# cgrigis/drynx

Hardware: AMD Instinct MI355X
Metric: end-to-end query latency + range-proof verifications/sec, logreg on 1e6 records (higher is better)
Workload: dtype bn254-exact/fp64

## Files before the change

### drynx_amd/native/__init__.py

```python
from __future__ import annotations

import ctypes
import os
import threading

import numpy as np

import torch

_HERE = os.path.dirname(os.path.abspath(__file__))
LIB_PATH = os.environ.get("DRYNX_NATIVE_LIB") or os.path.join(_HERE, "libdrynx_native.so")

_lib = None


def _load():
    global _lib
    if _lib is not None:
        return _lib
    if not os.path.exists(LIB_PATH):
        if os.environ.get("DRYNX_AUTOBUILD", "1") == "1":
            from . import build as _b

            _b.build()
        else:
            raise ImportError(f"{LIB_PATH} missing: run `python -m drynx_amd.native.build`")
    _lib = ctypes.CDLL(LIB_PATH)
    _declare(_lib)
    return _lib


_P = ctypes.c_void_p
_I = ctypes.c_int
_L = ctypes.c_int64

_SIGS = {
    "dx_fp_to_mont": [_I, _P, _P, _P, _L],
    "dx_fp_from_mont": [_I, _P, _P, _P, _L],
    "dx_fr_arith": [_I, _P, _I, _P, _P, _P, _L, _L],
    "dx_fr_dot_chunks": [_I, _P, _P, _P, _I, _P, _L, _L, _L],
    "dx_fr_seg_sum": [_I, _P, _P, _P, _P, _L],
    "dx_rp_challenges": [_I, _P, _P, _P, _P, _P, _P, _L],
    "dx_g1_fb_table": [_I, _P, _P, _P, _P, _L],
    "dx_g1_fb_mul": [_I, _P, _P, _P, _P, _L],
    "dx_g1_fb_mul_i64": [_I, _P, _P, _P, _P, _L],
    "dx_g1_fb_mul_idx": [_I, _P, _P, _P, _P, _P, _L],
    "dx_g1_mul": [_I, _P, _P, _P, _P, _L, _I, _I],
    "dx_g1_add": [_I, _P, _P, _P, _P, _L, _I, _I],
    "dx_g1_to_affine": [_I, _P, _P, _P, _L],
    "dx_g1_from_affine": [_I, _P, _P, _P, _L],
    "dx_g1_eq": [_I, _P, _P, _P, _P, _L],
    "dx_g1_on_curve": [_I, _P, _P, _P, _L],
    "dx_g1_sum_chunks": [_I, _P, _P, _P, _L, _L, _L],
    "dx_elgamal_encrypt": [_I, _P, _P, _P, _P, _P, _P, _P, _L],
    "dx_bsgs_build": [_I, _P, _P, _L, _P, _P, _L],
    "dx_bsgs_solve": [_I, _P, _P, _P, _P, _P, _L, _L, _L, _L, _P, _P, _L],
    "dx_g2_fb_table": [_I, _P, _P, _P, _P, _L],
    "dx_g2_fb_mul": [_I, _P, _P, _P, _P, _P, _L],
    "dx_g2_mul": [_I, _P, _P, _P, _P, _L, _I],
    "dx_g2_on_curve": [_I, _P, _P, _P, _L],
    "dx_miller_loop": [_I, _P, _P, _P, _P, _L],
    "dx_final_exp": [_I, _P, _P, _P, _L],
    "dx_pairing": [_I, _P, _P, _P, _P, _L],
    "dx_gt_mul": [_I, _P, _P, _P, _P, _L],
    "dx_gt_inv": [_I, _P, _P, _P, _L],
    "dx_prg_glv": [_I, _P, _P, ctypes.c_uint32, _P, _P, _P, _L],
    "dx_prg_bits": [_I, _P, _P, ctypes.c_uint32, _I, _P, _L],
    "dx_batched_copy": [_I, _P, _P, _P, _I, _L],
    "dx_copy_out": [_I, _P, _P, _P, _I, _L, _I],
    "dx_host_device_ptr": [_P, _P],
    "dx_rows_all": [_I, _P, _P, _P, _I, _L, _P],
    "dx_gt_pow": [_I, _P, _P, _P, _P, _L, _I],
    "dx_gt_eq": [_I, _P, _P, _P, _P, _L],
    "dx_gt_fb_table": [_I, _P, _P, _P, _P, _L],
    "dx_gt_fb_pow": [_I, _P, _P, _P, _P, _P, _L],
    "dx_gt_prod_chunks": [_I, _P, _P, _P, _L, _L, _L],
    "dx_version": [],
    "dx_lr_moments": [_P, _P, _P, _L, _I, _P, _I, _I],
    "dx_lr_gd_k2": [_P, _P, _P, _I, ctypes.c_double, ctypes.c_double, ctypes.c_double, _I, ctypes.c_double,
                    ctypes.c_double, ctypes.c_double, _P],
    "dx_random_scalars": [_I, _P, _P, ctypes.c_uint32, _P, _L],
    "dx_sha256_chunks": [_I, _P, _P, _L, _L, _P],
    "dx_hash_to_g1": [_I, _P, _P, _P, _L, _P, _L],
    "dx_lr_encode": [_P, _P, _L, _L, _I, _P, _P, _P, ctypes.c_double, ctypes.c_double, _P, _I, _I],
    "dx_lr_reduce": [_P, _P, _L, _L, _L, _P],
    "dx_lr_encode_upper": [_P, _P, _L, _L, _I, _P, _P, _P, ctypes.c_double, ctypes.c_double, _P, _I, _I],
    "dx_lr_reduce_pack": [_P, _P, _L, _I, _I, _L, ctypes.c_double, _P, _P],
    "dx_lr_encode_multi": [_P, _P, _L, _L, _I, _P, _P, _P, _L, _I, ctypes.c_double, _P, _I, _I, _I],
    "dx_lr_reduce_pack_multi": [_P, _P, _L, _I, _I, _I, _L, ctypes.c_double, _P, _P],
    "dx_g1_mul_glv256": [_P, _P, _P, _P, _P, _L, _I, _I, _I],
    "dx_glv_split": [_I, _P, _P, _P, _L],
    "dx_gt_t2_compress": [_I, _P, _P, _P, _P, _L],
    "dx_g2_x_compress": [_I, _P, _P, _P, _P, _P, _L],
    "dx_g2_x_decompress": [_I, _P, _P, _P, _P, _P, _L],
    "dx_gt_t2_decompress": [_I, _P, _P, _P, _L],
    "dx_gt_slice_prod": [_I, _P, _P, _P, _P, _P, _P, _L],
    "dx_gt_chunk_weight": [_I, _P, _P, _P, _P, _P, _P, _P, _L],
    "dx_g1_mul_glv": [_P, _P, _P, _P, _P, _L, _I],
    "dx_rp_u_joint_split": [_I, _P, _P, _P, _P, _L, _I, _I, _L, _I, _P, _P],
    "dx_bucket_bounds": [_I, _P, _P, _L, _L, _P, _P],
    "dx_slice_desc": [_I, _P, _P, _P, _P, _I, _L, _L, _P, _P],
    "dx_lane_slices": [_I, _P, _P, _P, _P, _P, _P, _L, _P, _P],
    "dx_g1_slice_sum": [_I, _P, _P, _P, _P, _P, _P, _L],
    "dx_rp_prove_a": [_I, _P, _P, _P, _P, _P, _P, _L, _I, _I],
    "dx_rp_prove_a_tab": [_I, _P, _P, _P, _P, _P, _P, _P, _L, _I, _I, _I],
    "dx_g2_fb4_table": [_I, _P, _P, _P, _P, _L],
    "dx_g2_fb4_mul": [_I, _P, _P, _P, _P, _P, _L],
    "dx_gt_fb4_table": [_I, _P, _P, _P, _P, _L],
    "dx_gt_fb4_pow": [_I, _P, _P, _P, _P, _P, _L],
    "dx_gt_cyclotomic": [_I, _P, _P, _P, _L],
    "dx_gt_membership": [_I, _P, _P, _P, _L],
    "dx_g1_horner_host": [_P, _P, _L, _I, _I],
    "dx_fp_sqrt_host": [_P, _P, _P, _P, _L],
    "dx_g2_chunk_weight": [_I, _P, _P, _P, _P, _P, _P, _P, _L],
    "dx_g2_subgroup": [_I, _P, _P, _P, _L],
    "dx_limbs_canonical": [_I, _P, _P, _I, _P, _L],
    "dx_g1j_on_curve": [_I, _P, _P, _P, _L],
    "dx_fold_steps": [],
    "dx_rp_coeffs": [_P, _P, _P, _L],
    "dx_int_moments": [_I, _P, _P, _L, _I, _P, _L, _P, _I, _P, _P],
    "dx_sha256_rows": [_I, _P, _P, _L, _L, _L, _L, _P],
    "dx_sha256_segments": [_I, _P, _P, _L, _L, _L, _P],
    "dx_g1_aff_to_uv": [_I, _P, _P, _L],
    "dx_rp_ncoeffs": [_P, _P, _P, _P, _L],
    "dx_rp_accum_n": [_P, _P, _P, _P, _P, _L, _L, _I, _I],
    "dx_ufold_coop_raw": [_P, _P, _P, _P, _P, _L, _L, _L],
    "dx_gt_frob8": [_I, _P, _P, _P, _L],
    "dx_gls6_entries": [],
    "dx_g2_gls6_table": [_I, _P, _P, _P, _P, _L],
    "dx_g2_gls6_mul": [_I, _P, _P, _P, _P, _P, _L],
    "dx_gt_gls6_table": [_I, _P, _P, _P, _P, _L],
    "dx_gt_gls6_pow": [_I, _P, _P, _P, _P, _P, _L],
    "dx_rp_prove_a_gls6": [_I, _P, _P, _P, _P, _P, _P, _P, _L, _I, _I],
    "dx_g2_joint_table": [_I, _P, _P, _P, _L],
    "dx_g2_joint_table_signed": [_I, _P, _P, _P, _P, _L],
    "dx_rp_u_group": [_I, _P, _P, _P, _P, _P, _P, _P, _L, _I, _L, _I, _I, _L, _P, _P],
    "dx_rp_u_joint": [_I, _P, _P, _P, _P, _L, _I, _I, _L, _P],
    "dx_g2_slice_sum": [_I, _P, _P, _P, _P, _P, _P, _L, _I, _L],
    "dx_g2_horner": [_I, _P, _P, _P, _I, _I, _I, _L, _L],
    "dx_rp_msm_uv": [_I, _P, _P, _P, _L, _I, _L],
    "dx_msm_keys": [_I, _P, _P, _P, _L, _L, _I, _I, _P, _P],
    "dx_gls8_entries": [],
    "dx_g2_gls8_table": [_I, _P, _P, _P, _P, _L],
    "dx_gt_gls8_table": [_I, _P, _P, _P, _P, _L, _P, _L],
    "dx_g2_gls8_mul": [_I, _P, _P, _P, _P, _P, _L],
    "dx_rp_prove_a_gls8": [_I, _P, _P, _P, _P, _P, _P, _P, _L, _I, _I, _I, _P],
    "dx_gt16_entries": [],
    "dx_gt16_table": [_I, _P, _P, _P, _P],
}


def _declare(lib):
    for name, args in _SIGS.items():
        fn = getattr(lib, name)
        fn.argtypes = args
        fn.restype = ctypes.c_int


def lib():
    return _load()


def loaded_path() -> str:
    _load()
    return LIB_PATH


_keep = threading.local()


def _ptr(t: torch.Tensor | None):
    if t is None:
        return None
    assert t.is_contiguous(), "native ops need contiguous tensors"
    held = getattr(_keep, "held", None)
    if held is None:
        held = _keep.held = []
    held.append(t)
    return ctypes.c_void_p(t.data_ptr())

# ... 1106 lines not shown
        raw = _bn.random_scalars(n, device)
    ab = raw[:, :2].contiguous()
    a = torch.zeros_like(raw)
    b = torch.zeros_like(raw)
    a[:, 0] = ab[:, 0]
    b[:, 0] = ab[:, 1]
    rho = fr_arith(FR_ADD, a, fr_arith(FR_MUL, b, _glv_const("lambda", device)))
    return ab, rho


def g1_mul_glv(pts_jac: torch.Tensor, ab: torch.Tensor) -> torch.Tensor:
    n = _rows(ab, 2)
    np_ = _rows(pts_jac, 24)
    assert np_ in (1, n)
    if not ab.is_cuda:
        a = torch.zeros((n, 8), dtype=torch.int32)
        b = torch.zeros((n, 8), dtype=torch.int32)
        a[:, 0], b[:, 0] = ab[:, 0], ab[:, 1]
        rho = fr_arith(FR_ADD, a, fr_arith(FR_MUL, b, _glv_const("lambda", "cpu")))
        return g1_mul(pts_jac, rho)
    out = torch.empty((n, 24), dtype=torch.int32, device=ab.device)
    _, s = _ctx(pts_jac, ab)
    rc = _raw_call("dx_g1_mul_glv", s, _ptr(pts_jac.contiguous()), _ptr(ab.contiguous()),
                   _ptr(_glv_const("beta", ab.device)), _ptr(out), n, int(np_ == 1 and n > 1))
    if rc:
        raise RuntimeError(f"dx_g1_mul_glv failed rc={rc}")
    return out


def g1_aff_to_uv_(aff: torch.Tensor) -> torch.Tensor:
    g, s = _ctx(aff)
    _call("dx_g1_aff_to_uv", g, s, _ptr(aff), _rows(aff, 16))
    return aff


FOLD_P_ALIGN = 8


def rp_fold_ncoeffs(V_aff: torch.Tensor) -> torch.Tensor:
    m = _rows(V_aff, 32)
    assert V_aff.is_cuda and V_aff.is_contiguous()
    steps = _load().dx_fold_steps()
    img = torch.empty((steps * 8 * m * 4,), dtype=torch.int32, device=V_aff.device)
    scratch = torch.empty((2 * steps * 4 * m * 4,), dtype=torch.int32, device=V_aff.device)
    _, s = _ctx(V_aff)
    _call("dx_rp_ncoeffs", s, _ptr(V_aff), _ptr(img), _ptr(scratch), m)
    return img


def rp_fold_accum_n(img: torch.Tensor, UV: torch.Tensor, V_aff: torch.Tensor, period: int, G: int,
                    K: int = 4) -> torch.Tensor:
    m = _rows(V_aff, 32)
    assert _rows(UV, 16) == G * period and period >= m and period % (64 * K * FOLD_P_ALIGN) == 0
    assert img.numel() == _load().dx_fold_steps() * 8 * m * 4
    fb = torch.empty((G * period // (64 * K), 96), dtype=torch.int32, device=UV.device)
    _, s = _ctx(img, UV, V_aff)
    _call("dx_rp_accum_n", s, _ptr(img), _ptr(UV), _ptr(V_aff), _ptr(fb), m, period, G, K)
    return fb


def rp_fold_accum_coop_raw(coef: torch.Tensor, P_aff: torch.Tensor, V_aff: torch.Tensor, period: int,
                           G: int) -> torch.Tensor:
    m = _rows(V_aff, 32)
    n = G * period
    assert _rows(P_aff, 16) == n and period >= m and period % 64 == 0
    assert coef.numel() == _load().dx_fold_steps() * 12 * m * 4
    f = torch.empty((n, 96), dtype=torch.int32, device=P_aff.device)
    _, s = _ctx(coef, P_aff, V_aff)
    _call("dx_ufold_coop_raw", s, _ptr(coef), _ptr(P_aff), _ptr(V_aff), _ptr(f), m, period, n)
    x = f.view(64, n // 64, 96)
    while x.shape[0] > 1:
        x = _gt_prod_level(x, 8)
    return x.view(n // 64, 96)


def gt_frob8(a: torch.Tensor, out: torch.Tensor | None = None) -> torch.Tensor:
    out = torch.empty_like(a) if out is None else out
    assert out.is_contiguous() and out.shape == a.shape
    g, s = _ctx(a)
    _call("dx_gt_frob8", g, s, _ptr(a.contiguous()), _ptr(out), _rows(a, 96))
    return out


def rp_fold_coeffs(V_aff: torch.Tensor) -> torch.Tensor:
    m = _rows(V_aff, 32)
    assert V_aff.is_cuda and V_aff.is_contiguous()
    coef = torch.empty((_load().dx_fold_steps() * 12 * m * 4,), dtype=torch.int32, device=V_aff.device)
    _, s = _ctx(V_aff)
    _call("dx_rp_coeffs", s, _ptr(V_aff), _ptr(coef), m)
    return coef


G2_JOINT_ENTRIES = 15


def g2_joint_table(V_aff: torch.Tensor, sign: torch.Tensor | None = None) -> torch.Tensor:
    m = _rows(V_aff, 32)
    out = torch.empty((m * G2_JOINT_ENTRIES, 32), dtype=torch.int32, device=V_aff.device)
    if sign is None:
        g, s = _ctx(V_aff)
        _call("dx_g2_joint_table", g, s, _ptr(V_aff.contiguous()), _ptr(out), m)
        return out
    assert sign.dtype == torch.int32 and sign.numel() == m
    g, s = _ctx(V_aff, sign)
    _call("dx_g2_joint_table_signed", g, s, _ptr(V_aff.contiguous()), _ptr(sign.contiguous()), _ptr(out), m)
    return out


def rp_u_joint(table: torch.Tensor, ab: torch.Tensor, n_groups: int, G: int, L: int, out: torch.Tensor,
               pad: int, pos: torch.Tensor | None = None) -> torch.Tensor:
    assert _rows(table, 32) == n_groups * L * G2_JOINT_ENTRIES and _rows(ab, 2) == G * n_groups * L
    assert out.is_contiguous() and pad >= n_groups
    if pos is None:
        assert _rows(out, 32) >= (G - 1) * pad + n_groups
    else:
        assert pos.dtype == torch.int64 and pos.numel() == G * n_groups and pos.device == out.device
    g, s = _ctx(table, ab, out)
    n = G * n_groups
    sp = 1 if (not g or n >= 131072) else (2 if n >= 65536 else 4)
    sp = min(sp, L)
    if sp > 1:
        tmp = torch.empty((n * sp, 48), dtype=torch.int32, device=out.device)
        _call("dx_rp_u_joint_split", g, s, _ptr(table), _ptr(ab.contiguous()), _ptr(out), n_groups, G, L, pad, sp,
              _ptr(tmp), _ptr(pos))
        return out
    _call("dx_rp_u_joint", g, s, _ptr(table), _ptr(ab.contiguous()), _ptr(out), n_groups, G, L, pad, _ptr(pos))
    return out


def rp_u_group_lanes(n: int, on_gpu: bool) -> int:
    if not on_gpu:
        return 1
    sp = 1
    while sp < 16 and n * sp < 32768:
        sp *= 2
    return sp


def rp_u_group(table: torch.Tensor, split: torch.Tensor, idx: torch.Tensor, start: torch.Tensor,
               length: torch.Tensor, G: int, nq: int, S: int, out: torch.Tensor, pad: int,
               pos: torch.Tensor | None = None, sp: int | None = None) -> torch.Tensor:
    ng = start.numel()
    assert _rows(table, 32) == G * nq * G2_JOINT_ENTRIES and _rows(split, 9) * S >= nq
    assert idx.dtype == torch.int32 and start.dtype == torch.int64 and length.dtype == torch.int32
    assert length.numel() == ng and out.is_contiguous() and pad >= ng
    if pos is None:
        assert _rows(out, 32) >= (G - 1) * pad + ng
    else:
        assert pos.dtype == torch.int64 and pos.numel() == G * ng and pos.device == out.device
    g, s = _ctx(table, split, idx, start, length, out)
    if sp is None:
        sp = rp_u_group_lanes(G * ng, bool(g))
    assert sp >= 1 and 64 % sp == 0
    tmp = None if g else torch.empty((G * ng * sp, 48), dtype=torch.int32)
    _call("dx_rp_u_group", g, s, _ptr(table), _ptr(split.contiguous()), _ptr(idx), _ptr(start), _ptr(length),
          _ptr(out), ng, G, nq, S, sp, pad, _ptr(pos), _ptr(tmp))
    return out


_gt_one_cache: dict = {}


def gt_one(device) -> torch.Tensor:
    key = str(device)
    if key not in _gt_one_cache:
        from ..crypto import bn254 as _bn

        t = np.zeros((1, 96), dtype=np.uint32)
        t[0, :8] = _bn.ints_to_limbs([_bn.mont(1)])[0]
        _gt_one_cache[key] = _bn.publish(_bn.to_tensor(t, device))
    return _gt_one_cache[key]


def _pow2_scalar(c: int) -> torch.Tensor:
    t = torch.zeros((1, 8), dtype=torch.int32)
    t[0, c // 32] = 1 << (c % 32)
    return t


def _finish_prod_on_host(parts: torch.Tensor) -> torch.Tensor:
    cur = parts.view(-1, 1, 96)
    while cur.shape[0] > 256:
        cur = _gt_prod_level(cur, 8)
    return gt_prod(cur.cpu(), chunk=4).view(1, 96)


def _gt_prod_level(x: torch.Tensor, ch: int) -> torch.Tensor:
    n_items, n_groups = x.shape[0], x.shape[1]
    n_chunks = (n_items + ch - 1) // ch
    out = torch.empty((n_chunks, n_groups, 96), dtype=torch.int32, device=x.device)
    g, s = _ctx(x)
    _call("dx_gt_prod_chunks", g, s, _ptr(x.contiguous()), _ptr(out), n_items, n_groups, ch)
    return out


from .msm import (G2_CHUNK, capture_keep, check_overflow, g1_msm, g1_msm_device, g1_msm_finish,
                  g1_msm_grouped, g1_msm_launch, g1_msm_plan, g1_slice_sum, g2_chunk_weight, g2_msm_device,
                  g2_msm_finish, g2_msm_launch, g2_msm_run, g2_slice_sum, gt_chunk_weight, gt_slice_prod, me_window,
                  multi_exp_device, multi_exp_grouped, multi_exp_grouped_finish, multi_exp_plan, rp_msm_uv)
```

### drynx_amd/native/msm.py

```python
from __future__ import annotations

import threading

import numpy as np

import torch

from . import (_call, _ctx, _gt_prod_level, _pow2_scalar, _ptr, _raw_call, _rows, _upload, g1_mul, gt_mul, gt_one,
               gt_pow, gt_prod)

_ME_SLICE = 8
G2_CHUNK = 32


def gt_slice_prod(src: torch.Tensor, idx, start: torch.Tensor, length: torch.Tensor) -> torch.Tensor:
    n = start.numel()
    out = torch.empty((n, 96), dtype=torch.int32, device=src.device)
    g, s = _ctx(src, idx, start, length)
    _call("dx_gt_slice_prod", g, s, _ptr(src), _ptr(idx), _ptr(start), _ptr(length), _ptr(out), n)
    return out


def g1_slice_sum(src: torch.Tensor, idx, start: torch.Tensor, length: torch.Tensor) -> torch.Tensor:
    n = start.numel()
    out = torch.empty((n, 24), dtype=torch.int32, device=src.device)
    g, s = _ctx(src, idx, start, length)
    _call("dx_g1_slice_sum", g, s, _ptr(src), _ptr(idx), _ptr(start), _ptr(length), _ptr(out), n)
    return out


def g2_slice_sum(src: torch.Tensor, idx, start: torch.Tensor, length: torch.Tensor, src_aff: bool,
                 idx_mod: int = 0) -> torch.Tensor:
    n = start.numel()
    assert src.shape[-1] == (32 if src_aff else 48) and (idx is None or idx.dtype == torch.int32)
    assert start.dtype == torch.int64 and length.dtype == torch.int32
    out = torch.empty((n, 48), dtype=torch.int32, device=src.device)
    g, s = _ctx(src, idx, start, length)
    _call("dx_g2_slice_sum", g, s, _ptr(src), _ptr(idx), _ptr(start), _ptr(length), _ptr(out), n, int(src_aff),
          int(idx_mod))
    return out


def gt_chunk_weight(B: torch.Tensor, d: torch.Tensor, start: torch.Tensor, length: torch.Tensor,
                    base: torch.Tensor) -> torch.Tensor:
    n = start.numel()
    out = torch.empty((n, 96), dtype=torch.int32, device=B.device)
    g, s = _ctx(B, d, start, length, base)
    _call("dx_gt_chunk_weight", g, s, _ptr(B.contiguous()), _ptr(d.contiguous()), _ptr(start), _ptr(length),
          _ptr(base), _ptr(out), n)
    return out


def g2_chunk_weight(B_jac: torch.Tensor, d: torch.Tensor, start: torch.Tensor, length: torch.Tensor,
                    base: torch.Tensor) -> torch.Tensor:
    n = start.numel()
    assert B_jac.shape[-1] == 48 and d.dtype == torch.int32 and start.dtype == torch.int64
    assert length.dtype == torch.int32 and base.dtype == torch.int32 and base.numel() == n
    out = torch.empty((n, 48), dtype=torch.int32, device=B_jac.device)
    g, s = _ctx(B_jac, d, start, length, base)
    _call("dx_g2_chunk_weight", g, s, _ptr(B_jac.contiguous()), _ptr(d.contiguous()), _ptr(start), _ptr(length),
          _ptr(base), _ptr(out), n)
    return out


def _gt_ops(a: torch.Tensor, items: torch.Tensor, item_split: tuple | None = None):
    n = a.shape[0]
    it = items.to(torch.int64)
    if item_split is not None:
        sp, q = item_split
        it = torch.where(it < sp, it % n, (it - sp) % q)
    else:
        it = it % n
    it = it.contiguous()
    return (lambda st, ln: gt_slice_prod(a, it, st, ln)), (lambda cur, st, ln: gt_slice_prod(cur, None, st, ln))


def _g1_ops(P_jac: torch.Tensor, items: torch.Tensor):
    P_jac, it = P_jac.contiguous(), items.to(torch.int64)
    return (lambda st, ln: g1_slice_sum(P_jac, it, st, ln)), (lambda cur, st, ln: g1_slice_sum(cur, None, st, ln))


def _g2_ops(P_aff: torch.Tensor, items: torch.Tensor, m: int):
    return (lambda st, ln: g2_slice_sum(P_aff, items, st, ln, True, m)), \
        (lambda cur, st, ln: g2_slice_sum(cur, None, st, ln, False))


def _group_arg(group, n: int, dev):
    if group is None:
        return None, 0
    if isinstance(group, int):
        return None, group
    assert group.numel() == n
    return group.to(device=dev, dtype=torch.int32).contiguous(), 0


def _runs(k: torch.Tensor, group, n_groups: int, W: int, c: int):
    dev = k.device
    n = k.shape[0]
    nb = (W << c) * n_groups
    assert n * W < 2 ** 31 and nb < 2 ** 31 - 1
    keys = torch.empty(n * W, dtype=torch.int32, device=dev)
    items = torch.empty(n * W, dtype=torch.int32, device=dev)
    grp, gstride = _group_arg(group, n, dev)
    g, s = _ctx(k, keys)
    _call("dx_msm_keys", g, s, _ptr(k.contiguous()), _ptr(grp), gstride, n, c, W, _ptr(keys), _ptr(items))
    k2, order = torch.sort(keys)
    items = items.index_select(0, order)
    bounds = torch.zeros((2, nb), dtype=torch.int64, device=dev)
    g, s = _ctx(k2)
    _call("dx_bucket_bounds", g, s, _ptr(k2), keys.numel(), nb, _ptr(bounds[0]), _ptr(bounds[1]))
    return items, bounds[0], bounds[1]


def _segment_passes(counts, first=None):
    passes = []
    c = np.asarray(counts, dtype=np.int64)
    while c.size and c.max() > 1:
        n_sl = (c + _ME_SLICE - 1) // _ME_SLICE
        if first is None:
            first = np.cumsum(c) - c
        b = np.repeat(np.arange(c.size), n_sl)
        k = np.arange(b.size) - (np.cumsum(n_sl) - n_sl)[b]
        passes.append((first[b] + k * _ME_SLICE, np.minimum(c[b] - k * _ME_SLICE, _ME_SLICE)))
        c, first = n_sl, None
    return passes


def _segment_passes_dev(counts, dev, first_slice: int | None = None):
    passes = []
    c = np.asarray(counts, dtype=np.int64)
    while c.size and c.max() > 1:
        sl = first_slice if (first_slice and not passes) else _ME_SLICE
        n_sl = (c + sl - 1) // sl
        total = int(n_sl.sum())
        meta = np.stack([np.cumsum(c) - c, c, np.cumsum(n_sl) - n_sl])
        m_dev = _upload(meta, dev)
        start = torch.empty(total, dtype=torch.int64, device=dev)
        ln = torch.empty(total, dtype=torch.int32, device=dev)
        g, s = _ctx(m_dev)
        _call("dx_slice_desc", g, s, _ptr(m_dev[0]), _ptr(m_dev[1]), _ptr(m_dev[2]), sl, c.size, total, _ptr(start),
              _ptr(ln))
        passes.append((start, ln))
        c = n_sl
    return passes


def _counted_plan(k: torch.Tensor, group, n_groups: int, W: int, c: int, first_slice: int | None = None) -> dict:
    dev = k.device
    items, first, end = _runs(k, group, n_groups, W, c)
    counts = (end - first).cpu().numpy().astype(np.int64)
    bk = np.flatnonzero(counts)
    passes = _segment_passes_dev(counts[bk], dev, first_slice)
    if bk.size and not passes:
        passes = [(torch.arange(bk.size, device=dev), torch.ones(bk.size, dtype=torch.int32, device=dev))]
    return {"item": items[: int(counts.sum())], "bk": bk, "passes": passes, "W": W, "c": c}


# ... 125 lines not shown
    gws, counts = np.unique(bk // 256, return_counts=True)
    return {"sc": _upload(sc, dev), "gws": gws,
            "passes": [(_upload(st, dev), _upload(ln.astype("int32"), dev)) for st, ln in _segment_passes(counts)]}


def _g1_weigh(h: dict, cur: torch.Tensor, wp: dict):
    cur = g1_mul(cur, wp["sc"])
    for st, ln in wp["passes"]:
        cur = g1_slice_sum(cur, None, st, ln)
    h["S_w"], h["gws"] = cur, wp["gws"]


def _g2_chunk(n_buckets: int) -> int:
    ch = G2_CHUNK
    while ch > 4 and n_buckets // ch < 16384:
        ch //= 2
    return ch


def _chunk_weight_plan(bk, c: int, dev) -> dict:
    chunk = _g2_chunk(bk.size)
    dig = bk & ((1 << c) - 1)
    gw = bk >> c
    ck = gw * ((1 << c) // chunk + 1) + dig // chunk
    first = np.flatnonzero(np.r_[True, ck[1:] != ck[:-1]])
    clen = np.diff(np.r_[first, bk.size])
    gwf = gw[first]
    gstart = np.flatnonzero(np.r_[True, gwf[1:] != gwf[:-1]])
    gws, gcounts = gwf[gstart], np.diff(np.r_[gstart, gwf.size])
    return {"d": _upload(dig.astype("int32"), dev),
            "chunks": (_upload(first.astype(np.int64), dev), _upload(clen.astype(np.int32), dev),
                       _upload(((dig[first] // chunk) * chunk).astype(np.int32), dev)),
            "gws": _upload(gws.astype(np.int64), dev), "gpasses": _segment_passes_dev(gcounts, dev)}


def _g2_weigh(cur, wp: dict, S: torch.Tensor) -> torch.Tensor:
    cur = g2_chunk_weight(cur, wp["d"], *wp["chunks"])
    for st, ln in wp["gpasses"]:
        cur = g2_slice_sum(cur, None, st, ln, False)
    S.index_copy_(0, wp["gws"], cur)
    return S


def _me_windows(h: dict, cur, bk, n_groups: int, W: int, c: int, dev):
    digit_sc = torch.zeros((bk.size, 8), dtype=torch.int32)
    digit_sc[:, 0] = torch.from_numpy((bk & ((1 << c) - 1)).astype("int32"))
    bkp = gt_pow(cur, _upload(digit_sc.numpy(), dev))
    D = 1 << c
    g, w, d = bk // (W * D), (bk >> c) % W, bk & (D - 1)
    slot = _upload(d * (n_groups * W) + g * W + w, dev)
    win = gt_one(dev).repeat(D * n_groups * W, 1)
    win[slot] = bkp
    win = win.view(D, n_groups * W, 96)
    if torch.device(dev).type == "cuda":
        while win.shape[0] > 32:
            win = _gt_prod_level(win, 8)
    h["win"] = win
    h["G"] = n_groups


def me_window(groups: tuple, lo: int = 8, hi: int = 16) -> tuple:
    def cost(c):
        return sum(r * -(-b // c) for r, b in groups) + 3 * sum(-(-b // c) for _, b in groups) * (1 << c)
    c = min(range(lo, hi + 1), key=cost)
    return max(-(-b // c) for _, b in groups), c


def multi_exp_plan(k: torch.Tensor, group, n_groups: int, W: int = 8, c: int = 8):
    return _counted_plan(k, group, n_groups, W, c)


def multi_exp_grouped(a: torch.Tensor, k: torch.Tensor, group, n_groups: int, W: int = 8, c: int = 8,
                      plan: dict | None = None):
    if plan is None:
        plan = _counted_plan(k, group, n_groups, W, c)
    h = {"G": n_groups, "W": W, "c": c, "win": None}
    if plan["bk"].size:
        cur = _reduce(plan["passes"], _gt_ops(a, plan["item"]))
        _me_windows(h, cur, plan["bk"], n_groups, W, c, a.device)
    return h


def multi_exp_device(a: torch.Tensor, k: torch.Tensor, group, groups: tuple, W: int | None = None,
                     c: int | None = None, item_split: tuple | None = None) -> dict:
    dev = a.device
    G = len(groups)
    if c is None:
        W, c = me_window(tuple(groups))
    B, lay, overflow = _device_buckets(k, group, groups, W, c, _ME_SLICE, lambda items: _gt_ops(a, items, item_split))
    if "gtw" not in lay:
        lay["gtw"] = _chunk_weight_plan(lay["used"], c, dev)
    wp = lay["gtw"]
    cur = gt_chunk_weight(B, wp["d"], *wp["chunks"])
    for st, ln in wp["gpasses"]:
        cur = gt_slice_prod(cur, None, st, ln)
    win = gt_one(dev).repeat(G * W, 1)
    win.index_copy_(0, wp["gws"], cur)
    return {"G": G, "W": W, "c": c, "win": win.view(1, G * W, 96), "overflow": overflow}


def multi_exp_grouped_finish(h) -> torch.Tensor:
    G, W = h["G"], h["W"]
    if h["win"] is None:
        return gt_one("cpu").repeat(G, 1)
    S_w = gt_prod(h["win"].cpu(), chunk=64).view(G, W, 96)
    acc = S_w[:, W - 1].contiguous()
    sh = _pow2_scalar(h["c"]).expand(G, 8).contiguous()
    for w in range(W - 2, -1, -1):
        acc = gt_mul(gt_pow(acc, sh), S_w[:, w].contiguous())
    return acc


def g1_msm(P_jac: torch.Tensor, k: torch.Tensor, bits: int = 256) -> torch.Tensor:
    return g1_msm_grouped(P_jac, k, None, 1, bits)


def g1_msm_grouped(P_jac: torch.Tensor, k: torch.Tensor, group: torch.Tensor | None, n_groups: int,
                   bits: int = 256) -> torch.Tensor:
    return g1_msm_finish(g1_msm_launch(P_jac, k, group, n_groups, bits))


def g1_msm_plan(k: torch.Tensor, group, n_groups: int, bits: int = 256):
    if not k.shape[0]:
        return None
    return _counted_plan(k, group, n_groups, (bits + 7) // 8, 8)


def g1_msm_launch(P_jac: torch.Tensor, k: torch.Tensor, group: torch.Tensor | None, n_groups: int,
                  bits: int = 256, plan: dict | None = None) -> dict:
    assert P_jac.shape[0] == k.shape[0]
    assert group is None or isinstance(group, int) or group.numel() == k.shape[0]
    W = (bits + 7) // 8
    h = {"n_groups": n_groups, "W": W, "S_w": None}
    if P_jac.shape[0] == 0:
        return h
    if plan is None:
        plan = _counted_plan(k, group, n_groups, W, 8)
    bk = plan["bk"]
    if bk.size:
        cur = _reduce(plan["passes"], _g1_ops(P_jac, plan["item"]))
        _g1_weigh(h, cur, _g1_weight_plan(bk, P_jac.device))
    return h


def g1_msm_device(P_jac: torch.Tensor, k: torch.Tensor, group, groups: tuple, bits: int = 256) -> dict:
    W = (bits + 7) // 8
    B, lay, overflow = _device_buckets(k, group, groups, W, 8, _ME_SLICE, lambda items: _g1_ops(P_jac, items))
    h = {"n_groups": len(groups), "W": W, "S_w": None, "overflow": overflow}
    if "g1w" not in lay:
        lay["g1w"] = _g1_weight_plan(lay["used"], P_jac.device)
    _g1_weigh(h, B, lay["g1w"])
    return h


def g1_msm_finish(h: dict) -> torch.Tensor:
    from ..crypto.bn254 import g1_infinity_jac

    out = g1_infinity_jac(h["n_groups"], "cpu")
    if h["S_w"] is None:
        return out
    W, gws = h["W"], h["gws"]
    S_w = h["S_w"].cpu()
    G = h["n_groups"]
    rows = g1_infinity_jac(G * W, "cpu")
    rows[torch.from_numpy(gws.astype(np.int64))] = S_w
    rows = rows.view(G, W, 24)
    top = int((gws % W).max())
    out = torch.empty((G, 24), dtype=torch.int32)
    src = rows[:, : top + 1].contiguous()
    rc = _raw_call("dx_g1_horner_host", _ptr(src), _ptr(out), G, top + 1, 8)
    if rc:
        raise RuntimeError(f"dx_g1_horner_host failed rc={rc}")
    return out


def g2_msm_launch(P_aff: torch.Tensor, k: torch.Tensor, group: torch.Tensor | None, n_groups: int,
                  c: int = 13, bits: int = 254, first_slice: int = 32):
    m = _rows(P_aff, 32)
    assert k.shape[0] % m == 0
    h = _counted_plan(k, group, n_groups, -(-bits // c), c, first_slice)
    h.update(G=n_groups, m=m)
    if h["bk"].size:
        h.update(_chunk_weight_plan(h["bk"], c, P_aff.device))
    return h


def g2_msm_run(P_aff: torch.Tensor, h: dict) -> torch.Tensor:
    S = torch.zeros((h["G"] * h["W"], 48), dtype=torch.int32, device=P_aff.device)
# ... 35 lines not shown
```

### drynx_amd/proofs/range_proof.py

```python
from __future__ import annotations

import hashlib
import io
import math
import os
import threading
from dataclasses import dataclass

import numpy as np
import torch

from .. import native as nt
from ..crypto import bn254 as bn
from ..crypto import oracle as O
from ..crypto.elgamal import CipherVector, pk_table
from ..query import PublishSignatureBytes
from ..utils import streams, timers
from ..utils.log import get_logger

log = get_logger("range_proof")

G2_LEN, G1_LEN, GT_LEN, SC_LEN = 128, 64, 384, 32


# ... 803 lines not shown
            dsc = torch.stack([wc.view(G, n, 8), w_all.view(G, n, 8)], 1).reshape(-1, 8).contiguous()
        if aux is None:
            S_R, hR = _pass_r(r.V, r.zphi, rho_all, meta)
        A2, mexp, e_all, dfull = _pass_me(r.A, ab_all, gam_all, rho_all, r.zv, w_all, r.zr, z, meta)
        with timers.span("rp.run.D"):
            if ddirect:
                if cC is None:
                    cC = nt.g1_mul(Cp.contiguous(), r.challenge.contiguous())
                elif ev_cC is not None:
                    torch.cuda.current_stream(device).wait_event(ev_cC)
                pts = torch.stack([cC, r.D], 1).unsqueeze(1).expand(n, G, 2, 24).reshape(-1, 24)
                abs_ = wab_all.view(G, n, 2).permute(1, 0, 2).unsqueeze(2).expand(n, G, 2, 2).reshape(-1, 2)
                dcheck = nt.g1_sum(nt.g1_mul_glv(pts.contiguous(), abs_.contiguous()).view(n, 2 * G, 24))
            else:
                dcheck = nt.g1_msm_device(dpts, dsc, n, ((n, 254),) * (2 * G))
    if aux is None:
        msq = _msm_queue(inp.get("Y", _inputs), r.V, ab_all, G, n, S, l, None, segs, ygroup=yg)
        for v, uok in zip(vns, msq["u_ok"]):
            v["u_ok"] = uok
    useg = fR = None
    with timers.span("rp.verify.multiexp"):
        if aux is not None:
            run_idle_tasks()
            ev_r.synchronize()
            with timers.span("rp.verify.r_tail"):
                fR, rok = _msm_r_miller(hR, S_R)
            ev_u.synchronize()
            with timers.span("rp.verify.u_tail"):
                useg = _seg_products(msq)
            aux.synchronize()
        GG = nt.multi_exp_grouped_finish(mexp)
        D_all = dcheck.cpu() if ddirect else nt.g1_msm_finish(dcheck)
        for h_ in (mexp, hR) if ddirect else (mexp, hR, dcheck):
            nt.check_overflow(h_)
        e_all, dfull = e_all.cpu(), dfull.cpu()
    with timers.span("rp.verify.fold_wait"):
        if useg is None:
            useg = _seg_products(msq)
        for k_, v in enumerate(vns):
            v["F"] = nt.gt_prod(useg[k_].view(-1, 1, 96), chunk=64).view(1, 96)
        if fR is None:
            fR, rok = _msm_r_miller(hR, S_R)
        for v, f, ok in zip(vns, fR, rok):
            v["F"], v["r_ok"] = nt.gt_mul(v["F"], f.view(1, 96)), ok
    for k, v in enumerate(vns):
        v.update(G=GG[k: k + 1], dfull=dfull[k], e=e_all[k: k + 1], dcheck=D_all[2 * k: 2 * k + 2])
    if vstream is not None:
        vstream.synchronize()
    if chk is not None:
        valid = valid & chk
    if vstream is not None:
        if not bool(valid.all()) and segs is None:
            return _invalid(valid, segs, n_vn)
    out = []
    m_oks = _gt_in_subgroup_each(GG[G: 2 * G])
    _, gt_tab = gt_generator_table("cpu")
    PB_base = bn.g1_jac_tensor([P_point, O.G1_GEN], "cpu")
    with timers.span("rp.verify.final_exp"):
        fe = nt.final_exp(torch.cat([v["F"].cpu().view(1, 96) for v in vns]).contiguous())
    for k_, v in enumerate(vns):
        with timers.span("rp.verify.finish"):
            G0 = v["dcheck"]
            PB = nt.g1_mul(PB_base, v["dfull"])
            v["dl"] = nt.g1_sum(torch.stack([G0[0:1], PB[0:1], PB[1:2]]))
            d_ok = bool(nt.g1_eq(v["dl"], G0[1:2])[0])
            v["lhs"] = lhs = nt.gt_mul(fe[k_: k_ + 1].contiguous(), v["G"].cpu())
            eq_ok = bool(nt.gt_eq(lhs, nt.gt_fb_pow(gt_tab, v["e"].cpu())).all())
        g2_ok = bool(v.get("u_ok", True)) and bool(v.get("r_ok", True))
        out.append(d_ok and m_oks[len(out)] and eq_ok and g2_ok)
        if not out[-1]:
            log.warning(f"range batch of {n} proofs failed for verifier {len(out) - 1}: D-check {d_ok}, "
                        f"GT membership {m_oks[len(out) - 1]}, pairing equation {eq_ok}, "
                        f"U in G2 {bool(v.get('u_ok', True))}, R in G2 {bool(v.get('r_ok', True))}")
    if segs is None:
        return out
    seg_valid = None if bool(valid.all()) else _seg_all(valid.view(1, -1), segs, valid.device).view(-1).tolist()
    redo = [k_ for k_ in range(G) if not out[k_] or (seg_valid is not None and not masked)]
    res = [([True] * nseg if seg_valid is None else list(seg_valid)) if ok else None for ok in out]
    if redo:
        if "items" in msq:
            with timers.span("rp.verify.useg_items"):
                useg = _useg_items(msq)
        with timers.span("rp.verify.segments"):
            x = dict(A2=A2, rho=rho_all, ab=ab_all, gam=gam_all, w=w_all, Cp=Cp, z=z, useg=useg, u_seg=msq["u_seg"],
                     PB_base=PB_base, gt_tab=gt_tab, wc=(4, 11) if device.type == "cuda" else wc_, G=G,
                     m_first=m_oks if seg_valid is None or masked else [False] * G,
                     tot=dict(lhs=[v.get("lhs") for v in vns], e=e_all, GGgam=GG[G: 2 * G],
                              dl=[v.get("dl") for v in vns], dr=[v["dcheck"][1:2] for v in vns],
                              r_ok=[bool(v.get("r_ok", True)) for v in vns]))
            if masked or seg_valid is None:
                per = _attribute_hinted(r, segs, redo, x)
            else:
                per = _segment_pass(r, segs, redo, x)
        for k_ in redo:
            if seg_valid is not None:
                per_k = [a and b for a, b in zip(per[k_], seg_valid)]
                res[k_] = None if masked and per_k == seg_valid else per_k
            else:
                res[k_] = per[k_] if not all(per[k_]) else None
    return res


_idle = threading.local()


class Deferred:

    def __init__(self, fn):
        self.fn, self.done, self.value = fn, False, None

    def run(self):
        if not self.done:
            self.value, self.done = self.fn(), True

    def result(self):
        self.run()
        return self.value


def add_idle_task(d: Deferred) -> Deferred:
    if not hasattr(_idle, "tasks"):
        _idle.tasks = []
    _idle.tasks.append(d)
    return d


def run_idle_tasks():
    tasks = getattr(_idle, "tasks", None)
    while tasks:
        tasks.pop(0).run()


class _nullctx:
    def __enter__(self):
        return self

    def __exit__(self, *a):
        return False


_SHAPE_INDEX: dict = {}
_SHAPE_INDEX_MAX = 16


def _shape_index(key, device, fn, n: int) -> torch.Tensor:
    k = (key, str(torch.device(device)))
    t = _SHAPE_INDEX.get(k)
    if t is None:
        if len(_SHAPE_INDEX) >= _SHAPE_INDEX_MAX:
            if torch.device(device).type == "cuda":
                torch.cuda.synchronize(device)
            _SHAPE_INDEX.clear()
        t = _SHAPE_INDEX[k] = bn.publish(fn(torch.arange(n, device=device)).contiguous())
    if t.is_cuda:
        t.record_stream(torch.cuda.current_stream(t.device))
    return t


def _pass_r(V, zphi, rho, meta):
    G, m, S, l, gb, wc, cR = meta
    zi = _shape_index(("zphi", m, S, l), V.device,
                      lambda it: (it // (S * l)) * l + it % l, m)
    s_r = nt.fr_arith(nt.FR_MUL, rho, zphi.index_select(0, zi).contiguous())
    with timers.span("rp.run.R"):
        return nt.g2_msm_device(V, s_r, m, ((m, 254),) * G, c=cR)


def _pass_me(A, ab, gam, rho, zv, w, zr, z, meta):
    G, m, S, l, gb, wc, cR = meta
    dev = A.device
    with timers.span("rp.frob8"):
        A2 = torch.empty((2 * m, 96), dtype=torch.int32, device=dev)
        A2[:m].copy_(A)
        nt.gt_frob8(A.contiguous(), out=A2[m:])
    abv = ab.view(G, m, 2)
    k = torch.zeros((3 * G * m, 8), dtype=torch.int32, device=dev)
    kr = k[: 2 * G * m].view(G, 2 * m, 8)
    kr[:, :m, 0] = abv[:, :, 0]
    kr[:, m:, 0] = abv[:, :, 1]
    k[2 * G * m:] = gam
    mgrp = _shape_index(("mgrp", G, m), dev,
                        lambda e: torch.where(e < 2 * G * m, e // (2 * m), G + (e - 2 * G * m) // m).to(torch.int32),
                        3 * G * m)
    with timers.span("rp.run.ME"):
        mexp = nt.multi_exp_device(A2, k, mgrp, ((2 * m, 32),) * G + ((m, gb),) * G, wc[0], wc[1],
                                   item_split=(2 * G * m, m))
    e_all = nt.fr_dot_rows(rho, zv, G, b_periodic=True)
    dfull = torch.stack([nt.fr_dot_rows(w, zr, G, b_periodic=True),
                         nt.fr_dot_rows(w, z, G, b_periodic=True)], 1)
    return A2, mexp, e_all, dfull


_DCHECK_DIRECT_MAX = 16384


def _r_window(m: int, G: int) -> int:
    return min(range(8, 14), key=lambda c: -(-254 // c) * (m + 8 * (1 << c)))


_YGROUP_MIN_MULT = 3
_KEY_GROUPS: dict = {}
_KEY_GROUPS_MAX = 8


def _key_groups(cols, S: int, n_cols: int, device) -> dict:
    dev = torch.device(device)
    c = np.asarray(cols, dtype=np.int64)
    k = (c.tobytes(), S, n_cols, str(dev))
    kg = _KEY_GROUPS.get(k)
    if kg is None:
        if len(_KEY_GROUPS) >= _KEY_GROUPS_MAX:
            if dev.type == "cuda":
                torch.cuda.synchronize(dev)
            _KEY_GROUPS.clear()
        y_idx = (np.arange(S).reshape(1, S) * n_cols + c.reshape(-1, 1)).reshape(-1)
        keys, inv = np.unique(y_idx, return_inverse=True)
        inv = inv.reshape(-1)
        ln = np.bincount(inv, minlength=len(keys))
        ts = [_h2d(np.argsort(inv, kind="stable").astype(np.int32), dev),
              _h2d((np.cumsum(ln) - ln).astype(np.int64), dev), _h2d(ln.astype(np.int32), dev),
              _h2d(keys.astype(np.int64), dev)]
        bn.publish(ts)
        kg = _KEY_GROUPS[k] = dict(idx=ts[0], start=ts[1], len=ts[2], keys=ts[3], ng=len(keys))
    if dev.type == "cuda":
        for t in (kg["idx"], kg["start"], kg["len"], kg["keys"]):
            t.record_stream(torch.cuda.current_stream(dev))
    return kg


def _msm_queue(Y, V, ab_all, G: int, n: int, S: int, L: int, vstream=None, segs: list | None = None,
               table=None, ygroup: dict | None = None) -> dict:
    dev = V.device
    nq = n * S
    qoff = np.cumsum([0] + [c * S for c in segs]) if segs else np.array([0, nq])
    cq = np.diff(qoff)
    if table is None:
        with timers.span("rp.u.joint_table"):
            table = nt.g2_joint_table(V)
    out = {"G": G}
    lay = pos = None
    if dev.type == "cuda" and ygroup is None:
        lay = _fold_layout(G, nq, cq, dev)
        pad, pos = lay["pad"], lay["pos"]
        Uall = torch.zeros((G * pad, 32), dtype=torch.int32, device=dev)
    else:
        pad = nq
        Uall = torch.zeros((G * nq, 32), dtype=torch.int32, device=dev)
    with timers.span("rp.u.joint"):
        nt.rp_u_joint(table, ab_all, nq, G, L, Uall, pad, pos)
    if dev.type == "cuda":
        cur = torch.cuda.current_stream(dev)
        vs = vstream if vstream is not None else cur
        vs.wait_stream(cur)
        with torch.cuda.stream(vs):
            flags = nt.g2_subgroup(Uall)
            fl = (flags.view(G, pad)[:, :nq] if pos is None else flags.index_select(0, pos).view(G, nq)).bool()
            out["u_seg"] = _seg_all(fl, cq, dev)
            out["u_ok"] = list(out["u_seg"].all(dim=1).unbind(0))
        Uall.record_stream(vs)
        if pos is not None:
            pos.record_stream(vs)
    else:
        out["u_seg"] = _seg_all(nt.g2_subgroup(Uall).view(G, nq).bool(), cq, dev)
        out["u_ok"] = [bool(x) for x in out["u_seg"].all(dim=1).tolist()]
    if ygroup is not None:
        kg = ygroup["groups"]
        ng = kg["ng"]
        with timers.span("rp.u.group"):
# ... 379 lines not shown
```

Measured before the change: 394,500.

## Use compressed torus representation for GT multi-exponentiation bucket products

GT elements for the range-proof multi-exponentiation are converted to a compressed torus form (one Fp6 per row, with batched inversion across chunks of rows). Bucket slice products then run on these half-size elements using paired-thread torus multiplication. The result is decompressed on the host after the window products. The first-level slice length rises from 8 to 32. This halves memory traffic and cuts per-multiply cost, in exchange for an extra inversion pass, special handling of degenerate rows, and a decompression step. The old frob8 stacking is now built lazily only when segment attribution needs it.

```diff
diff --git a/csrc/kernels/dx_me_torus.hip b/csrc/kernels/dx_me_torus.hip
--- /dev/null
+++ b/csrc/kernels/dx_me_torus.hip
@@ -0,0 +1,136 @@
+#define DX_NI __host__ __device__ __forceinline__
+#include "common.h"
+#include "../bn254/gt_torus.h"
+
+using namespace dxk;
+
+namespace {
+constexpr int kWG = 64;
+namespace tp = torus::pair;
+
+DX_HD Fp6 canon6(const Fp6 &h) {
+  auto c2 = [](const Fp2 &a) { return Fp2{reduce_256<FpParams>(a.c0.v), reduce_256<FpParams>(a.c1.v)}; };
+  return {c2(h.c0), c2(h.c1), c2(h.c2)};
+}
+
+DX_HD Fp6 frob8_image(const Fp6 &b) {
+  return {dx::mul(b.c0, Fp2::from_limbs(Frob::G2[2])), dx::mul(b.c1, Fp2::from_limbs(Frob::G2[4])), b.c2};
+}
+
+DX_HD bool is_skip_row(const Fp6 &b) {
+  const uint32_t *w = &b.c0.c0.v[0];
+  uint32_t acc = 0;
+#pragma unroll
+  for (int i = 0; i < 48; i++) acc |= w[i];
+  return acc == 0;
+}
+
+DX_HD void beta_rows_chunk(const uint32_t *a, uint32_t *beta2, int64_t m, int64_t i0, int64_t i1) {
+  Fp6 acc = Fp6::one();
+  for (int64_t i = i0; i < i1; i++) {
+    const Fp6 h = canon6(at<Fp12>(a, i).c1);
+    at<Fp6>(beta2, i) = acc;
+    if (!(h == Fp6::zero())) acc = torus::mul6(acc, h);
+  }
+  Fp6 inv_all = inv(acc);
+  for (int64_t i = i1 - 1; i >= i0; i--) {
+    const Fp6 h = canon6(at<Fp12>(a, i).c1);
+    if (h == Fp6::zero()) {
+      at<Fp6>(beta2, i) = Fp6::zero();
+      at<Fp6>(beta2, m + i) = Fp6::zero();
+      continue;
+    }
+    const Fp6 hi = torus::mul6(inv_all, at<Fp6>(beta2, i));
+    inv_all = torus::mul6(inv_all, h);
+    const Fp6 b = torus::mul6(add(Fp6::one(), at<Fp12>(a, i).c0), hi);
+    at<Fp6>(beta2, i) = b;
+    at<Fp6>(beta2, m + i) = frob8_image(b);
+  }
+}
+
+__global__ void __launch_bounds__(kWG) DX_OCC gt_beta_rows_kernel(const uint32_t *a, uint32_t *beta2, int64_t m,
+                                                                 int64_t k, int64_t chunks) {
+  const int64_t t = (int64_t)blockIdx.x * kWG + threadIdx.x;
+  if (t >= chunks) return;
+  const int64_t i0 = t * k, i1 = i0 + k < m ? i0 + k : m;
+  beta_rows_chunk(a, beta2, m, i0, i1);
+}
+
+__global__ void __launch_bounds__(kWG) DX_OCC gt_beta_slice_prod_pair(const uint32_t *beta, const int64_t *idx,
+                                                                     const int64_t *start, const int32_t *len,
+                                                                     uint32_t *out, int64_t n_slices) {
+  const tp::Role R = tp::role();
+  const int64_t s = (int64_t)blockIdx.x * tp::kPairs + R.g;
+  if (s >= n_slices) return;
+  const int64_t b = start[s];
+  const int n = len[s];
+  const Fp6 *T = reinterpret_cast<const Fp6 *>(beta);
+  Fp6 x = tp::one(R);
+  int k = 0;
+  for (; k < n; k++) {
+    const Fp6 bt = T[idx ? idx[b + k] : b + k];
+    if (is_skip_row(bt)) continue;
+    x = tp::sel6(R.r != 0, Fp6::one(), bt);
+    k++;
+    break;
+  }
+  for (; k < n; k++) {
+    const Fp6 bt = T[idx ? idx[b + k] : b + k];
+    if (!is_skip_row(bt)) tp::mul_beta(x, bt, false, R);
+  }
+  tp::store(&at<Fp12>(out, s), x, R);
+}
+
+inline dim3 grid_of(int64_t n) { return dim3((unsigned)((n + kWG - 1) / kWG)); }
+inline dim3 grid_pair(int64_t n) { return dim3((unsigned)((n + tp::kPairs - 1) / tp::kPairs)); }
+}
+
+extern "C" {
+int dx_gt_beta_rows(int on_gpu, void *stream, const uint32_t *a, uint32_t *beta2, int64_t m, int64_t rows_per_inv) {
+  if (m <= 0) return 0;
+  const int64_t k = rows_per_inv < 1 ? 1 : rows_per_inv;
+  const int64_t chunks = (m + k - 1) / k;
+  if (!on_gpu) {
+    host_for_each(chunks, [=](int64_t t) {
+      const int64_t i0 = t * k, i1 = i0 + k < m ? i0 + k : m;
+      beta_rows_chunk(a, beta2, m, i0, i1);
+    }, 2);
+    return 0;
+  }
+  hipLaunchKernelGGL(gt_beta_rows_kernel, grid_of(chunks), dim3(kWG), 0, (hipStream_t)stream, a, beta2, m, k, chunks);
+  return check_hip(hipGetLastError(), "gt_beta_rows");
+}
+
+int dx_gt_beta_slice_prod(int on_gpu, void *stream, const uint32_t *beta, const int64_t *idx, const int64_t *start,
+                          const int32_t *len, uint32_t *out, int64_t n_slices) {
+  if (n_slices <= 0) return 0;
+  if (!on_gpu) {
+    host_for_each(n_slices, [=](int64_t s) {
+      const int64_t b = start[s];
+      const int n = len[s];
+      Fp12 y = Fp12::one();
+      bool have = false;
+      for (int k = 0; k < n; k++) {
+        const Fp6 bt = at<Fp6>(beta, idx ? idx[b + k] : b + k);
+        if (is_skip_row(bt)) continue;
+        if (have) {
+          torus::mul_beta(y, bt, false);
+        } else {
+          y = Fp12{bt, Fp6::one()};
+          have = true;
+        }
+      }
+      at<Fp12>(out, s) = y;
+    });
+    return 0;
+  }
+  hipLaunchKernelGGL(gt_beta_slice_prod_pair, grid_pair(n_slices), dim3(kWG), 0, (hipStream_t)stream, beta, idx,
+                     start, len, out, n_slices);
+  return check_hip(hipGetLastError(), "gt_beta_slice_prod");
+}
+
+int dx_gt_pi(int on_gpu, void *stream, const uint32_t *y, uint32_t *out, int64_t n) {
+  auto op = [=] __host__ __device__(int64_t i) { at<Fp12>(out, i) = torus::finish(at<Fp12>(y, i)); };
+  return run(on_gpu, stream, n, op, true, "gt_pi");
+}
+}
diff --git a/drynx_amd/native/__init__.py b/drynx_amd/native/__init__.py
--- a/drynx_amd/native/__init__.py
+++ b/drynx_amd/native/__init__.py
@@ -96,6 +96,9 @@
     "dx_gt_t2_decompress": [_I, _P, _P, _P, _L],
     "dx_gt_slice_prod": [_I, _P, _P, _P, _P, _P, _P, _L],
     "dx_gt_chunk_weight": [_I, _P, _P, _P, _P, _P, _P, _P, _L],
+    "dx_gt_beta_rows": [_I, _P, _P, _P, _L, _L],
+    "dx_gt_beta_slice_prod": [_I, _P, _P, _P, _P, _P, _P, _L],
+    "dx_gt_pi": [_I, _P, _P, _P, _L],
     "dx_g1_mul_glv": [_P, _P, _P, _P, _P, _L, _I],
     "dx_rp_u_joint_split": [_I, _P, _P, _P, _P, _L, _I, _I, _L, _I, _P, _P],
     "dx_bucket_bounds": [_I, _P, _P, _L, _L, _P, _P],
@@ -1368,6 +1371,23 @@
     return out
 
 
+def gt_beta_rows(a: torch.Tensor, rows_per_inv: int | None = None) -> torch.Tensor:
+    m = _rows(a, 96)
+    if rows_per_inv is None:
+        rows_per_inv = 8 if a.device.type != "cuda" else max(1, min(8, m // (1024 * 64 * 2)))
+    out = torch.empty((2 * m, 48), dtype=torch.int32, device=a.device)
+    g, s = _ctx(a)
+    _call("dx_gt_beta_rows", g, s, _ptr(a.contiguous()), _ptr(out), m, int(rows_per_inv))
+    return out
+
+
+def gt_pi(y: torch.Tensor) -> torch.Tensor:
+    out = torch.empty_like(y)
+    g, s = _ctx(y)
+    _call("dx_gt_pi", g, s, _ptr(y.contiguous()), _ptr(out), _rows(y, 96))
+    return out
+
+
 def rp_fold_coeffs(V_aff: torch.Tensor) -> torch.Tensor:
     m = _rows(V_aff, 32)
     assert V_aff.is_cuda and V_aff.is_contiguous()
@@ -1482,5 +1502,6 @@
 
 from .msm import (G2_CHUNK, capture_keep, check_overflow, g1_msm, g1_msm_device, g1_msm_finish,
                   g1_msm_grouped, g1_msm_launch, g1_msm_plan, g1_slice_sum, g2_chunk_weight, g2_msm_device,
-                  g2_msm_finish, g2_msm_launch, g2_msm_run, g2_slice_sum, gt_chunk_weight, gt_slice_prod, me_window,
-                  multi_exp_device, multi_exp_grouped, multi_exp_grouped_finish, multi_exp_plan, rp_msm_uv)
+                  g2_msm_finish, g2_msm_launch, g2_msm_run, g2_slice_sum, gt_beta_slice_prod, gt_chunk_weight,
+                  gt_slice_prod, me_window, multi_exp_device, multi_exp_grouped, multi_exp_grouped_finish,
+                  multi_exp_plan, rp_msm_uv)
diff --git a/drynx_amd/native/msm.py b/drynx_amd/native/msm.py
--- a/drynx_amd/native/msm.py
+++ b/drynx_amd/native/msm.py
@@ -7,9 +7,10 @@
 import torch
 
 from . import (_call, _ctx, _gt_prod_level, _pow2_scalar, _ptr, _raw_call, _rows, _upload, g1_mul, gt_mul, gt_one,
-               gt_pow, gt_prod)
+               gt_pi, gt_pow, gt_prod)
 
 _ME_SLICE = 8
+_ME_TORUS_SLICE = 32
 G2_CHUNK = 32
 
 
@@ -18,6 +19,16 @@
     out = torch.empty((n, 96), dtype=torch.int32, device=src.device)
     g, s = _ctx(src, idx, start, length)
     _call("dx_gt_slice_prod", g, s, _ptr(src), _ptr(idx), _ptr(start), _ptr(length), _ptr(out), n)
+    return out
+
+
+def gt_beta_slice_prod(beta: torch.Tensor, idx, start: torch.Tensor, length: torch.Tensor) -> torch.Tensor:
+    n = start.numel()
+    assert beta.shape[-1] == 48 and (idx is None or idx.dtype == torch.int64)
+    assert start.dtype == torch.int64 and length.dtype == torch.int32
+    out = torch.empty((n, 96), dtype=torch.int32, device=beta.device)
+    g, s = _ctx(beta, idx, start, length)
+    _call("dx_gt_beta_slice_prod", g, s, _ptr(beta), _ptr(idx), _ptr(start), _ptr(length), _ptr(out), n)
     return out
 
 
@@ -65,6 +76,7 @@
 
 def _gt_ops(a: torch.Tensor, items: torch.Tensor, item_split: tuple | None = None):
     n = a.shape[0]
+    first = gt_beta_slice_prod if a.shape[-1] == 48 else gt_slice_prod
     it = items.to(torch.int64)
     if item_split is not None:
         sp, q = item_split
@@ -72,7 +84,7 @@
     else:
         it = it % n
     it = it.contiguous()
-    return (lambda st, ln: gt_slice_prod(a, it, st, ln)), (lambda cur, st, ln: gt_slice_prod(cur, None, st, ln))
+    return (lambda st, ln: first(a, it, st, ln)), (lambda cur, st, ln: gt_slice_prod(cur, None, st, ln))
 
 
 def _g1_ops(P_jac: torch.Tensor, items: torch.Tensor):
@@ -364,12 +376,14 @@
 
 
 def multi_exp_device(a: torch.Tensor, k: torch.Tensor, group, groups: tuple, W: int | None = None,
-                     c: int | None = None, item_split: tuple | None = None) -> dict:
+                     c: int | None = None, item_split: tuple | None = None, first_slice: int | None = None) -> dict:
     dev = a.device
+    torus = a.shape[-1] == 48
+    sl = first_slice or (_ME_TORUS_SLICE if torus else _ME_SLICE)
     G = len(groups)
     if c is None:
         W, c = me_window(tuple(groups))
-    B, lay, overflow = _device_buckets(k, group, groups, W, c, _ME_SLICE, lambda items: _gt_ops(a, items, item_split))
+    B, lay, overflow = _device_buckets(k, group, groups, W, c, sl, lambda items: _gt_ops(a, items, item_split))
     if "gtw" not in lay:
         lay["gtw"] = _chunk_weight_plan(lay["used"], c, dev)
     wp = lay["gtw"]
@@ -378,14 +392,17 @@
         cur = gt_slice_prod(cur, None, st, ln)
     win = gt_one(dev).repeat(G * W, 1)
     win.index_copy_(0, wp["gws"], cur)
-    return {"G": G, "W": W, "c": c, "win": win.view(1, G * W, 96), "overflow": overflow}
+    return {"G": G, "W": W, "c": c, "win": win.view(1, G * W, 96), "overflow": overflow, "torus": torus}
 
 
 def multi_exp_grouped_finish(h) -> torch.Tensor:
     G, W = h["G"], h["W"]
     if h["win"] is None:
         return gt_one("cpu").repeat(G, 1)
-    S_w = gt_prod(h["win"].cpu(), chunk=64).view(G, W, 96)
+    S_w = gt_prod(h["win"].cpu(), chunk=64)
+    if h.get("torus"):
+        S_w = gt_pi(S_w)
+    S_w = S_w.view(G, W, 96)
     acc = S_w[:, W - 1].contiguous()
     sh = _pow2_scalar(h["c"]).expand(G, 8).contiguous()
     for w in range(W - 2, -1, -1):
diff --git a/drynx_amd/proofs/range_proof.py b/drynx_amd/proofs/range_proof.py
--- a/drynx_amd/proofs/range_proof.py
+++ b/drynx_amd/proofs/range_proof.py
@@ -909,6 +909,8 @@
             with timers.span("rp.verify.useg_items"):
                 useg = _useg_items(msq)
         with timers.span("rp.verify.segments"):
+            if A2 is None:
+                A2 = _stack_frob8(r.A)
             x = dict(A2=A2, rho=rho_all, ab=ab_all, gam=gam_all, w=w_all, Cp=Cp, z=z, useg=useg, u_seg=msq["u_seg"],
                      PB_base=PB_base, gt_tab=gt_tab, wc=(4, 11) if device.type == "cuda" else wc_, G=G,
                      m_first=m_oks if seg_valid is None or masked else [False] * G,
@@ -993,13 +995,28 @@
         return nt.g2_msm_device(V, s_r, m, ((m, 254),) * G, c=cR)
 
 
+_ME_TORUS_DEFAULT = "1"
+
+
+def _me_torus() -> bool:
+    return os.environ.get("DRYNX_ME_TORUS", _ME_TORUS_DEFAULT) == "1"
+
+
+def _stack_frob8(A: torch.Tensor) -> torch.Tensor:
+    m = A.shape[0]
+    A2 = torch.empty((2 * m, 96), dtype=torch.int32, device=A.device)
+    A2[:m].copy_(A)
+    nt.gt_frob8(A.contiguous(), out=A2[m:])
+    return A2
+
+
 def _pass_me(A, ab, gam, rho, zv, w, zr, z, meta):
     G, m, S, l, gb, wc, cR = meta
     dev = A.device
+    torus = _me_torus()
     with timers.span("rp.frob8"):
-        A2 = torch.empty((2 * m, 96), dtype=torch.int32, device=dev)
-        A2[:m].copy_(A)
-        nt.gt_frob8(A.contiguous(), out=A2[m:])
+        A2 = None if torus else _stack_frob8(A)
+        src = nt.gt_beta_rows(A) if torus else A2
     abv = ab.view(G, m, 2)
     k = torch.zeros((3 * G * m, 8), dtype=torch.int32, device=dev)
     kr = k[: 2 * G * m].view(G, 2 * m, 8)
@@ -1010,7 +1027,7 @@
                         lambda e: torch.where(e < 2 * G * m, e // (2 * m), G + (e - 2 * G * m) // m).to(torch.int32),
                         3 * G * m)
     with timers.span("rp.run.ME"):
-        mexp = nt.multi_exp_device(A2, k, mgrp, ((2 * m, 32),) * G + ((m, gb),) * G, wc[0], wc[1],
+        mexp = nt.multi_exp_device(src, k, mgrp,((2 * m, 32),) * G + ((m, gb),) * G, wc[0], wc[1],
                                    item_split=(2 * G * m, m))
     e_all = nt.fr_dot_rows(rho, zv, G, b_periodic=True)
     dfull = torch.stack([nt.fr_dot_rows(w, zr, G, b_periodic=True),
```

Result: faster. 416,200, median of 6 (+5.5%).
